# daovietanh190499/3D_Reconstruction

Measured on AMD Instinct MI355X. Metric: image-pairs matched/sec, higher is better.
Workload: dtype f32 descriptors: int8 MFMA certified filter + f64 re-score; 1 GPU; C3/C4 all-pairs BF-L2 + ratio 0.75: 257 imgs x 4096 kpts x 256-d, exact f32-input semantics (oracle.match.bf_match_exact, bit for bit); pairs=32896, api=dist.match_all_pairs_sharded(exact=True), match_mode=exact-float, parallelism=pairs/1

## Files before the change

### 3d_reconstruction_amd/csrc/match.hip

```cpp
#include "common.h"
#include <climits>
#include <cstdlib>

namespace sfmhip {

typedef int i32x4 __attribute__((ext_vector_type(4)));
typedef int i32x16 __attribute__((ext_vector_type(16)));

constexpr int kJB = 128;

template <int D>
__device__ __forceinline__ int swz_off(int r, int c) {
    constexpr int CPR = D / 16;
    constexpr int RPB = 256 / D;
    return r * D + ((c ^ ((r / RPB) % CPR)) << 4);
}

__device__ __forceinline__ int max3i(int a, int b, int c) {
    int r;
    asm("v_max3_i32 %0, %1, %2, %3" : "=v"(r) : "v"(a), "v"(b), "v"(c));
    return r;
}
__device__ __forceinline__ int med3i(int a, int b, int c) {
    int r;
    asm("v_med3_i32 %0, %1, %2, %3" : "=v"(r) : "v"(a), "v"(b), "v"(c));
    return r;
}

__global__ void quantize_kernel(const float* __restrict__ in, int64_t total, int d, int m_pad,
                                const int32_t* __restrict__ nk, int mode, int8_t* __restrict__ out) {
    const int64_t n4 = total >> 2;
    for (int64_t q = (int64_t)blockIdx.x * blockDim.x + threadIdx.x; q < n4;
         q += (int64_t)gridDim.x * blockDim.x) {
        const int64_t e = q << 2;
        const int64_t row = e / d;
        const int img = (int)(row / m_pad);
        const int r = (int)(row % m_pad);
        const float4 x = *reinterpret_cast<const float4*>(in + e);
        char4 o = make_char4(0, 0, 0, 0);
        if (r < nk[img]) {
            float v[4] = {x.x, x.y, x.z, x.w};
            int qv[4];
#pragma unroll
            for (int t = 0; t < 4; ++t) {
                if (mode == 0) {
                    float rr = fminf(fmaxf(__builtin_rintf(v[t]), 0.f), 255.f);
                    qv[t] = (int)rr - 128;
                } else {
                    float rr = __builtin_rintf(127.f * v[t]);
                    rr = fminf(fmaxf(rr, -127.f), 127.f);
                    qv[t] = (int)rr;
                }
            }
            o = make_char4((signed char)qv[0], (signed char)qv[1], (signed char)qv[2], (signed char)qv[3]);
        }
        *reinterpret_cast<char4*>(out + e) = o;
    }
}

__global__ void prepare_kernel(const int8_t* __restrict__ desc, int n_rows, int m_pad, int d,
                               const int32_t* __restrict__ nk, int32_t* __restrict__ norms,
                               int32_t* __restrict__ keys) {
    const int row = blockIdx.x * blockDim.x + threadIdx.x;
    if (row >= n_rows) return;
    const int img = row / m_pad, r = row % m_pad;
    const int8_t* p = desc + (size_t)row * d;
    int s = 0;
    for (int k = 0; k < d; k += 16) {
        const i32x4 v = *reinterpret_cast<const i32x4*>(p + k);
#pragma unroll
        for (int w = 0; w < 4; ++w) {
            const int x = v[w];
#pragma unroll
            for (int t = 0; t < 4; ++t) {
                const int q = (int)(signed char)((x >> (8 * t)) & 0xff);
                s += q * q;
            }
        }
    }
    norms[row] = s;
    const int low = 127 - (r & (kJB - 1));
    keys[row] = (r < nk[img]) ? (-s * 128 + low) : (INT_MIN + low);
}

__global__ void key_values_kernel(const int32_t* __restrict__ keys, int64_t n, int32_t* __restrict__ h,
                                  float* __restrict__ hf) {
    for (int64_t e = (int64_t)blockIdx.x * blockDim.x + threadIdx.x; e < n; e += (int64_t)gridDim.x * blockDim.x) {
        const int v = keys[e] >> 8;
        h[e] = v;
        if (hf) hf[e] = (float)v;
    }
}

__device__ __forceinline__ int fp6_grid_index(float y, int* g) {
    const float t = fminf(fabsf(y), 60.f);
    int n, m;
    if (t < 16.f) { m = (int)__builtin_rintf(t); n = m; }
    else if (t < 32.f) { const int r = (int)__builtin_rintf(0.5f * t); m = 2 * r; n = r + 8; }
    else { const int r = (int)__builtin_rintf(0.25f * t); m = 4 * r; n = r + 16; }
    const bool neg = y < 0.f && m > 0;
    *g = neg ? -m : m;
    return n | (neg ? 32 : 0);
}
__global__ void quantize_fp6_kernel(const float* __restrict__ in, int64_t n_chunks, int d, int m_pad,
                                    const int32_t* __restrict__ nk, int8_t* __restrict__ g,
                                    uint8_t* __restrict__ code) {
    for (int64_t c = (int64_t)blockIdx.x * blockDim.x + threadIdx.x; c < n_chunks;
         c += (int64_t)gridDim.x * blockDim.x) {
        const int64_t e0 = c * 32, row = e0 / d;
        const int img = (int)(row / m_pad), r = (int)(row % m_pad);
        const bool valid = r < nk[img];
        unsigned gw[8], cw[8];
#pragma unroll
        for (int w = 0; w < 8; ++w) gw[w] = cw[w] = 0u;
        if (valid) {
#pragma unroll
            for (int q = 0; q < 8; ++q) {
                const float4 x = *reinterpret_cast<const float4*>(in + e0 + 4 * q);
                const float v[4] = {x.x, x.y, x.z, x.w};
                unsigned pk = 0u;
#pragma unroll
                for (int t = 0; t < 4; ++t) {
                    int gv;
                    const int cd = fp6_grid_index(127.f * v[t], &gv);
                    gw[q] |= (unsigned)(gv & 0xff) << (8 * t);
                    pk |= (unsigned)cd << (6 * t);
                }
#pragma unroll
                for (int t = 0; t < 3; ++t) {
                    const int byte = 3 * q + t;
                    cw[byte >> 2] |= ((pk >> (8 * t)) & 0xffu) << (8 * (byte & 3));
                }
            }
        }
        uint4* go = reinterpret_cast<uint4*>(g + e0);
        uint4* co = reinterpret_cast<uint4*>(code + e0);
        go[0] = make_uint4(gw[0], gw[1], gw[2], gw[3]);
        go[1] = make_uint4(gw[4], gw[5], gw[6], gw[7]);
        co[0] = make_uint4(cw[0], cw[1], cw[2], cw[3]);
        co[1] = make_uint4(cw[4], cw[5], cw[6], cw[7]);
    }
}

template <int D, int WAVES>
struct Stager {
    static constexpr int CPR = D / 16;
    static constexpr int RPB = 256 / D;
    static constexpr int TILE = kJB * D;
    static constexpr int NI = TILE / 1024;
    static constexpr int PER_WAVE = NI / WAVES;
    static constexpr int LDT = TILE / 16 / (64 * WAVES);
    static_assert(NI % WAVES == 0 && LDT >= 1, "block / workgroup mismatch");

    __device__ static void dma(const int8_t* src, const int32_t* ksrc, int8_t* dst, int32_t* kdst, int wave,
                               int lane) {
#pragma unroll
        for (int u = 0; u < PER_WAVE; ++u) {
            const int ins = wave * PER_WAVE + u;
            const int rows_per_ins = 1024 / D;
            const int r0 = ins * rows_per_ins;
            const int r = r0 + lane / CPR;
            const int c = (lane % CPR) ^ ((r / RPB) % CPR);
            __builtin_amdgcn_global_load_lds(
                (__attribute__((address_space(1))) void*)(src + (size_t)r * D + c * 16),
                (__attribute__((address_space(3))) void*)(dst + r0 * D), 16, 0, 0);
        }
        if (wave == WAVES - 1) {
#pragma unroll
            for (int u = 0; u < 2; ++u)
                __builtin_amdgcn_global_load_lds(
                    (__attribute__((address_space(1))) void*)(ksrc + u * 64 + lane),
                    (__attribute__((address_space(3))) void*)(kdst + u * 64), 4, 0, 0);
        }
    }
};

template <int MF> struct Mfma;
template <> struct Mfma<32> {
    using acc_t = i32x16;
    static constexpr int NREG = 16, KB = 32;
    __device__ static acc_t run(i32x4 a, i32x4 b, acc_t c) {
        return __builtin_amdgcn_mfma_i32_32x32x32_i8(a, b, c, 0, 0, 0);
    }
    __device__ static int row(int q, int grp) { return (q & 3) + 8 * (q >> 2) + 4 * grp; }
};
template <> struct Mfma<16> {
    using acc_t = i32x4;
    static constexpr int NREG = 4, KB = 64;
    __device__ static acc_t run(i32x4 a, i32x4 b, acc_t c) {
        return __builtin_amdgcn_mfma_i32_16x16x64_i8(a, b, c, 0, 0, 0);
    }
    __device__ static int row(int q, int grp) { return 4 * grp + q; }
};

struct CertArgs {
    const double* erow;
    const double* eimg;
    double inv_s;
    int force;
};
constexpr int kUndecidedBase = -3;
constexpr int kValueOnlyTiles = 4;
__device__ __forceinline__ int sqrt8_ceil(int d2) {
    const long long t = 64LL * d2;
    int u = (int)ceil(sqrt((double)t));
    while (u > 0 && (long long)(u - 1) * (u - 1) >= t) --u;
    while ((long long)u * u < t) ++u;
    return u;
}
template <typename OutT>
__device__ __forceinline__ int undecided_mark(int d2) {
    if constexpr (sizeof(OutT) == 2) return kUndecidedBase - sqrt8_ceil(d2);
    else return kUndecidedBase - d2;
}
template <typename OutT>
__device__ __forceinline__ double mark_sqrt_d2(int mark) {
    if constexpr (sizeof(OutT) == 2) return (double)(kUndecidedBase - mark) * 0.125;
    else return sqrt((double)(kUndecidedBase - mark));
}

__device__ __forceinline__ int certify(int d1lo, int d1hi, int d2lo, int d2hi, double E, double inv_s, double rn2,
                                       double rd2) {
    const double up = 1.0 + 0x1p-50, dn = 1.0 - 0x1p-50;
    const double s1l = sqrt((double)d1lo) * inv_s, s1h = sqrt((double)d1hi) * inv_s;
    const double s2l = sqrt((double)d2lo) * inv_s, s2h = sqrt((double)d2hi) * inv_s;
    const double a1 = fmax(s1l * dn - E * up, 0.0), b1 = (s1h + E) * up;
    const double a2 = fmax(s2l * dn - E * up, 0.0), b2 = (s2h + E) * up;
    const double wl = 1.0 - 1e-12, wh = 1.0 + 1e-12;
    const double lo1 = a1 * a1 * wl, hi1 = b1 * b1 * wh, lo2 = a2 * a2 * wl, hi2 = b2 * b2 * wh;
    if (rd2 * lo1 >= rn2 * hi2) return 0;
    if (hi1 < lo2 && rd2 * hi1 < rn2 * lo2) return 1;
    return -1;
}

template <int D, int MF, int NS, int VG, typename OutT>
__device__ __forceinline__ void value_only_tail(const int (&w1)[NS], const int (&w2)[NS], const int (&wr)[NS],
                                                const int8_t* __restrict__ desc, const int8_t* __restrict__ bdesc,
                                                const int32_t* __restrict__ bkeys, const int32_t* __restrict__ norms,
                                                int a, int b, int m_pad, int na_rows, int ibase, int grp, int lr,
                                                int lane, long long rn2, long long rd2, OutT* __restrict__ out_m,
                                                const CertArgs& ca) {
    constexpr int NG = 64 / MF;
    int v1 = INT_MIN, v2 = INT_MIN, loc = 0;
#pragma unroll
    for (int s = 0; s < NS; ++s) {
        int a1 = w1[s], a2 = w2[s], al = wr[s] * NG + grp;
#pragma unroll
        for (int off = MF; off < 64; off <<= 1) {
            const int o1 = __shfl_xor(a1, off), o2 = __shfl_xor(a2, off), ol = __shfl_xor(al, off);
            const bool mine = a1 > o1 || (a1 == o1 && al < ol);
            a2 = max3i(min(a1, o1), a2, o2);
            al = mine ? al : ol;
            a1 = max(a1, o1);
        }
        if (s == grp) { v1 = a1; v2 = a2; loc = al; }
    }
    const int i = ibase + grp * MF + lr;
    int res = -1, na = 0, du1 = 0, hidx = -1;
    double E = 0.0;
    bool survivor = false;
    if (i < na_rows) {
        na = norms[(size_t)a * m_pad + i];
        du1 = na - 2 * v1;
        const int du2ub = na - 2 * v2;
        E = ca.erow[(size_t)a * m_pad + i] + ca.eimg[b];
        if (ca.force)
            res = undecided_mark<OutT>(min(du2ub, D * 255 * 255));
        else
            survivor = certify(max(du1 - 1, 0), du1, max(du1 - 1, 0), du2ub, E, ca.inv_s, (double)rn2,
                               (double)rd2) != 0;
    }
    constexpr int NC = 4 * VG;
    constexpr int LPC = (64 / NC) < (D / 16) ? (64 / NC) : (D / 16);
    constexpr int BPL = D / LPC;
    const int c = min(lane / LPC, NC - 1), part = lane % LPC;
    unsigned long long bal = __ballot(survivor);
    while (bal) {
        const int l = __builtin_ctzll(bal);
        bal &= bal - 1;
        const int ri = __shfl(i, l), rv = __shfl(v1, l), rl = __shfl(loc, l);
        const int j0 = (rl / NG) * VG * MF + 4 * (rl % NG);
        const int j = j0 + (c >> 2) * MF + (c & 3);
        const int8_t* pa = desc + ((size_t)a * m_pad + ri) * D + part * BPL;
        const int8_t* pb = bdesc + (size_t)j * D + part * BPL;
        int dot = 0;
#pragma unroll
        for (int w = 0; w < BPL / 16; ++w) {
            const i32x4 x = *reinterpret_cast<const i32x4*>(pa + 16 * w);
            const i32x4 y = *reinterpret_cast<const i32x4*>(pb + 16 * w);
#pragma unroll
            for (int e = 0; e < 4; ++e) dot = __builtin_amdgcn_sdot4(x[e], y[e], dot, false);
        }
#pragma unroll
        for (int off = 1; off < LPC; off <<= 1) dot += __shfl_xor(dot, off);
        const int u = dot + bkeys[j];
        const bool hit = lane < NC * LPC && part == 0 && u == rv;
        const unsigned long long hb = __ballot(hit);
        int x = u == rv ? INT_MIN : u;
#pragma unroll
        for (int off = LPC; off < 64; off <<= 1) x = max(x, __shfl_xor(x, off));
        if (lane == l) {
            const bool one = __popcll(hb) == 1;
            v2 = max(v2, one ? x : rv);
            if (one) {
                const int hc = __builtin_ctzll(hb) / LPC;
                hidx = j0 + (hc >> 2) * MF + (hc & 3);
            }
        }
    }
    if (survivor) {
        const int du2 = na - 2 * v2;
        const int v = certify(max(du1 - 1, 0), du1, max(du2 - 1, 0), du2, E, ca.inv_s, (double)rn2, (double)rd2);
        res = v == 0 ? -1 : (v > 0 && hidx >= 0) ? hidx : undecided_mark<OutT>(du2);
    }
    if (i < m_pad) out_m[i] = (OutT)res;
}

template <int D, int MF, int NS, int WAVES, bool CERT = false, typename OutT = int32_t, int VG = 0>
__global__ __launch_bounds__(64 * WAVES, 2) void match_kernel(
    const int8_t* __restrict__ desc, const int32_t* __restrict__ norms,
    const int32_t* __restrict__ keys, const int32_t* __restrict__ nk, int m_pad,
    const int32_t* __restrict__ pairs, int n_iblk, int nwg, long long rn2, long long rd2,
    OutT* __restrict__ m0, int32_t* __restrict__ dist1, int32_t* __restrict__ dist2, CertArgs ca) {
    using S = Stager<D, WAVES>;
    using M = Mfma<MF>;
    using acc_t = typename M::acc_t;
    constexpr int KK = D / M::KB;
    constexpr int CPK = M::KB / 16;
    constexpr int NG = 64 / MF;
    constexpr int TILE = S::TILE;
    constexpr int NT = 64 * WAVES;
    constexpr int IW = MF * NS;
    constexpr int IB = IW * WAVES;
    constexpr int JT = kJB / MF;
    static_assert(NS % NG == 0 || NG % NS == 0, "output lane mapping");
    constexpr bool VO = VG > 0;
    static_assert(!VO || (CERT && M::NREG == 4 && NS == NG && JT % VG == 0), "value-only form: 16x16 tiles, NS == NG");

    __shared__ __attribute__((aligned(16))) int8_t lds[2 * TILE + 2 * kJB * 4];

    const int wg = xcd_remap(blockIdx.x, nwg);
    const int pair = wg / n_iblk, ib = wg % n_iblk;
    const int a = pairs[2 * pair], b = pairs[2 * pair + 1];
    const int na_rows = nk[a], nb_rows = nk[b];
    const int tid = threadIdx.x, lane = tid & 63;
    const int wave = __builtin_amdgcn_readfirstlane(tid >> 6);
    const int grp = lane / MF, lr = lane % MF;
    const int ibase = ib * IB + wave * IW;
    OutT* out_m = m0 + (size_t)pair * m_pad;

    if (ib * IB >= na_rows || nb_rows < 2) {
        const int iend = min(ib * IB + IB, m_pad);
        for (int i = ib * IB + tid; i < iend; i += NT) {
            out_m[i] = -1;
            if (dist1) dist1[(size_t)pair * m_pad + i] = -1;
            if (dist2) dist2[(size_t)pair * m_pad + i] = -1;
        }
        return;
    }

    const int8_t* bdesc = desc + (size_t)b * m_pad * D;
    const int32_t* bkeys = keys + (size_t)b * m_pad;
    const int nblk = (nb_rows + kJB - 1) / kJB;
    int32_t* kbase = reinterpret_cast<int32_t*>(lds + 2 * TILE);

    S::dma(bdesc, bkeys, lds, kbase, wave, lane);

    i32x4 bq[NS][KK];
#pragma unroll
    for (int s = 0; s < NS; ++s) {
        const int i = min(ibase + s * MF + lr, m_pad - 1);
        const int8_t* rp = desc + ((size_t)a * m_pad + i) * D + grp * 16;
#pragma unroll
        for (int kk = 0; kk < KK; ++kk) bq[s][kk] = *reinterpret_cast<const i32x4*>(rp + kk * M::KB);
    }

    int g1k[NS], g1i[NS], g2k[NS], g1w[NS], g1b[NS];
#pragma unroll
    for (int s = 0; s < NS; ++s) { g1k[s] = INT_MIN; g1i[s] = 0; g1w[s] = 127; g1b[s] = 0; g2k[s] = INT_MIN; }
    int w1[NS], w2[NS], wr[NS];
#pragma unroll
    for (int s = 0; s < NS; ++s) { w1[s] = INT_MIN; w2[s] = INT_MIN; wr[s] = 0; }

    __syncthreads();

    for (int blk = 0; blk < nblk; ++blk) {
        const int cur = blk & 1;
        if (blk + 1 < nblk)
            S::dma(bdesc + (size_t)(blk + 1) * TILE, bkeys + (blk + 1) * kJB, lds + (cur ^ 1) * TILE,
                   kbase + (cur ^ 1) * kJB, wave, lane);
        const int8_t* tl = lds + cur * TILE;
        const int32_t* kl = kbase + cur * kJB;
        if constexpr (VO) {
            int rm[NS];
#pragma unroll
            for (int jt = 0; jt < JT; ++jt) {
                if (jt % VG == 0) {
#pragma unroll
                    for (int s = 0; s < NS; ++s) rm[s] = INT_MIN;
                }
                const i32x4 hv = *reinterpret_cast<const i32x4*>(kl + jt * MF + M::row(0, grp));
                acc_t acc[NS];
#pragma unroll
                for (int s = 0; s < NS; ++s) acc[s] = hv;
                const int r = jt * MF + lr;
#pragma unroll
                for (int kk = 0; kk < KK; ++kk) {
                    const i32x4 av = *reinterpret_cast<const i32x4*>(tl + swz_off<D>(r, kk * CPK + grp));
#pragma unroll
                    for (int s = 0; s < NS; ++s) acc[s] = M::run(av, bq[s][kk], acc[s]);
                }
#pragma unroll
                for (int s = 0; s < NS; ++s) {
                    rm[s] = max(max(rm[s], acc[s][0]), acc[s][1]);
                    rm[s] = max(max(rm[s], acc[s][2]), acc[s][3]);
                }
                if (jt % VG == VG - 1) {
                    const int rid = blk * (JT / VG) + jt / VG;
#pragma unroll
                    for (int s = 0; s < NS; ++s) {
                        wr[s] = rm[s] > w1[s] ? rid : wr[s];
                        w2[s] = med3i(w1[s], w2[s], rm[s]);
                        w1[s] = max(w1[s], rm[s]);
                    }
                }
            }
            __syncthreads();
            continue;
        }
        int t1[NS], t2[NS];
#pragma unroll
        for (int s = 0; s < NS; ++s) { t1[s] = INT_MIN; t2[s] = INT_MIN; }
#pragma unroll
        for (int jt = 0; jt < JT; ++jt) {
            acc_t acc[NS];
#pragma unroll
            for (int s = 0; s < NS; ++s) acc[s] = acc_t{0};
            const int r = jt * MF + lr;
#pragma unroll
            for (int kk = 0; kk < KK; ++kk) {
                const i32x4 av = *reinterpret_cast<const i32x4*>(tl + swz_off<D>(r, kk * CPK + grp));
#pragma unroll
                for (int s = 0; s < NS; ++s) acc[s] = M::run(av, bq[s][kk], acc[s]);
            }
#pragma unroll
            for (int g = 0; g < M::NREG / 4; ++g) {
                const i32x4 kv = *reinterpret_cast<const i32x4*>(kl + jt * MF + M::row(4 * g, grp));
#pragma unroll
                for (int e = 0; e < 4; e += 2) {
#pragma unroll
                    for (int s = 0; s < NS; ++s) {
                        const int ka = acc[s][4 * g + e] * 256 + kv[e];
                        const int kb = acc[s][4 * g + e + 1] * 256 + kv[e + 1];
                        const int m = med3i(t1[s], ka, kb);
                        t1[s] = max3i(t1[s], ka, kb);
                        t2[s] = max(t2[s], m);
                    }
                }
            }
        }
#pragma unroll
        for (int s = 0; s < NS; ++s) {
            if constexpr (D <= 128) {
                const int k1 = t1[s] >> 7, k2 = t2[s] >> 7;
                const bool up = k1 > g1k[s];
                g2k[s] = max3i(min(g1k[s], k1), g2k[s], k2);
                g1w[s] = up ? t1[s] : g1w[s];
                g1b[s] = up ? blk : g1b[s];
                g1k[s] = max(g1k[s], k1);
            } else {
                const int k1 = t1[s] >> 7, k2 = t2[s] >> 7, ix = blk * kJB + 127 - (t1[s] & 127);
                if (k1 > g1k[s]) { g2k[s] = max(g1k[s], k2); g1k[s] = k1; g1i[s] = ix; }
                else             { g2k[s] = max(g2k[s], k1); }
            }
        }
        __syncthreads();
    }

    if constexpr (VO) {
        value_only_tail<D, MF, NS, VG, OutT>(w1, w2, wr, desc, bdesc, bkeys, norms, a, b, m_pad, na_rows, ibase, grp, lr,
                                             lane, rn2, rd2, out_m, ca);
        return;
    }
    if constexpr (D <= 128) {
#pragma unroll
        for (int s = 0; s < NS; ++s) g1i[s] = g1b[s] * kJB + 127 - (g1w[s] & 127);
    }
#pragma unroll
    for (int s = 0; s < NS; ++s) {
#pragma unroll
        for (int off = MF; off < 64; off <<= 1) {
            const int ok = __shfl_xor(g1k[s], off), oi = __shfl_xor(g1i[s], off), o2 = __shfl_xor(g2k[s], off);
            const bool mine = (g1k[s] > ok) || (g1k[s] == ok && g1i[s] < oi);
            const int n2 = mine ? max(g2k[s], ok) : max(o2, g1k[s]);
            if (!mine) { g1k[s] = ok; g1i[s] = oi; }
            g2k[s] = n2;
        }
    }
#pragma unroll
    for (int s = 0; s < NS; ++s) {
        if (s % NG != grp % NS) continue;
        const int i = ibase + s * MF + lr;
        if (i >= m_pad) continue;
        int res = -1, d1 = -1, d2 = -1;
        if (i < na_rows) {
            const int na = norms[(size_t)a * m_pad + i];
            d1 = na - g1k[s];
            d2 = na - g2k[s];
            if (CERT) {
                const int v = ca.force ? -1
                                       : certify(d1, d1, d2, d2, ca.erow[(size_t)a * m_pad + i] + ca.eimg[b], ca.inv_s,
                                                 (double)rn2, (double)rd2);
                res = v > 0 ? g1i[s] : (v == 0 ? -1 : undecided_mark<OutT>(d2));
            } else if (rd2 * (long long)d1 < rn2 * (long long)d2) {
                res = g1i[s];
            }
        }
        out_m[i] = (OutT)res;
        if (dist1) dist1[(size_t)pair * m_pad + i] = d1;
        if (dist2) dist2[(size_t)pair * m_pad + i] = d2;
    }
}

typedef int i32x2 __attribute__((ext_vector_type(2)));
typedef int i32x8 __attribute__((ext_vector_type(8)));
typedef float f32x4 __attribute__((ext_vector_type(4)));

__global__ void pack_fp6_kernel(const uint8_t* __restrict__ code, int64_t n_chunks, int d,
                                uint8_t* __restrict__ dense) {
    const int spr = d / 32;
    for (int64_t c = (int64_t)blockIdx.x * blockDim.x + threadIdx.x; c < n_chunks;
         c += (int64_t)gridDim.x * blockDim.x) {
        const int64_t row = c / spr;
        const int s = (int)(c % spr);
        const uint4 lo = *reinterpret_cast<const uint4*>(code + c * 32);
        const uint2 hi = *reinterpret_cast<const uint2*>(code + c * 32 + 16);
        uint8_t* rp = dense + row * (3 * d / 4);
        *reinterpret_cast<uint4*>(rp + 16 * s) = lo;
        *reinterpret_cast<uint2*>(rp + d / 2 + 8 * s) = hi;
    }
}

template <int D, int WAVES>
struct DenseStager {
    static constexpr int ROW = 3 * D / 4, LB = D / 2, HB = D / 4;
    static constexpr int LO = kJB * LB, TILE = kJB * ROW;
    static constexpr int CPR = LB / 16, RPB = 256 / LB;
    static constexpr int UPR = HB / 16, RPH = 256 / HB;
    static constexpr int NLO = LO / 1024 / WAVES, NHI = (TILE - LO) / 1024 / WAVES;
    static_assert(NLO * WAVES * 1024 == LO && NHI * WAVES * 1024 == TILE - LO && NLO >= 1 && NHI >= 1,
                  "block / workgroup mismatch");
    static_assert(RPB * CPR == 16 && RPH * UPR == 16, "a 16-row tile covers every bank once");

    __device__ static int lo_sw(int r) { return ((((r & 15) + 4) >> 3) & 1) ^ ((r / RPB) % CPR); }
    __device__ static int hi_sw(int r) { return (r / RPH) % UPR; }
    __device__ static int lo_off(int r, int s) { return r * LB + ((s ^ lo_sw(r)) << 4); }
    __device__ static int hi_off(int r, int s) { return LO + r * HB + ((((s >> 1) ^ hi_sw(r)) << 4) | ((s & 1) << 3)); }

    __device__ static void dma(const uint8_t* src, const int32_t* ksrc, int8_t* dst, int32_t* kdst, int wave,
                               int lane) {
#pragma unroll
        for (int u = 0; u < NLO; ++u) {
            const int ins = wave * NLO + u;
            const int r = ins * (1024 / LB) + lane / CPR;
            const int c = (lane % CPR) ^ lo_sw(r);
            __builtin_amdgcn_global_load_lds(
                (__attribute__((address_space(1))) void*)(src + (size_t)r * ROW + c * 16),
                (__attribute__((address_space(3))) void*)(dst + ins * 1024), 16, 0, 0);
        }
#pragma unroll
        for (int u = 0; u < NHI; ++u) {
            const int ins = wave * NHI + u;
            const int r = ins * (1024 / HB) + lane / UPR;
            const int c = (lane % UPR) ^ hi_sw(r);
            __builtin_amdgcn_global_load_lds(
                (__attribute__((address_space(1))) void*)(src + (size_t)r * ROW + LB + c * 16),
                (__attribute__((address_space(3))) void*)(dst + LO + ins * 1024), 16, 0, 0);
        }
        if (wave == WAVES - 1) {
#pragma unroll
            for (int u = 0; u < 2; ++u)
                __builtin_amdgcn_global_load_lds(
                    (__attribute__((address_space(1))) void*)(ksrc + u * 64 + lane),
                    (__attribute__((address_space(3))) void*)(kdst + u * 64), 4, 0, 0);
        }
    }
};

__device__ __forceinline__ i32x2 lds_read_b64(const int8_t* p) {
    return *(const volatile __attribute__((address_space(3))) i32x2*)p;
}

struct Fp6Operand {
    i32x4 lo;
    i32x2 hi;
    __device__ i32x8 tuple() const { return i32x8{lo[0], lo[1], lo[2], lo[3], hi[0], hi[1], 0, 0}; }
};

constexpr int kFp6Tiles = 8;
constexpr int kFp6Waves = 4;

template <int D, typename OutT>
__global__ __launch_bounds__(64 * kFp6Waves, 2) void match_fp6_kernel(
    const uint8_t* __restrict__ dense, const int8_t* __restrict__ g, const int32_t* __restrict__ norms,
    const int32_t* __restrict__ h, const float* __restrict__ hf, const int32_t* __restrict__ nk, int m_pad,
    const int32_t* __restrict__ pairs, int n_iblk, int nwg, long long rn2, long long rd2,
    OutT* __restrict__ m0, CertArgs ca) {
    constexpr int MF = 16, NS = kFp6Tiles, WAVES = kFp6Waves, VG = kValueOnlyTiles;
    static_assert(D % 128 == 0, "one scaled MFMA takes 128 elements of k");
    static_assert(NS % 4 == 0, "value_only_tail takes four query tiles at a time");
    using S = DenseStager<D, WAVES>;
    constexpr int KK = D / 128;
    constexpr int TILE = S::TILE;
    constexpr int NT = 64 * WAVES;
    constexpr int IW = MF * NS, IB = IW * WAVES;
    constexpr int JT = kJB / MF;
    constexpr int kScale = (int)0x82828282;
    constexpr float kLow = -16777216.f;

    __shared__ __attribute__((aligned(16))) int8_t lds[2 * TILE + 2 * kJB * 4];

    const int wg = xcd_remap(blockIdx.x, nwg);
    const int pair = wg / n_iblk, ib = wg % n_iblk;
    const int a = pairs[2 * pair], b = pairs[2 * pair + 1];
    const int na_rows = nk[a], nb_rows = nk[b];
    const int tid = threadIdx.x, lane = tid & 63;
    const int wave = __builtin_amdgcn_readfirstlane(tid >> 6);
    const int grp = lane / MF, lr = lane % MF;
    const int ibase = ib * IB + wave * IW;
    OutT* out_m = m0 + (size_t)pair * m_pad;

    if (ib * IB >= na_rows || nb_rows < 2) {
        const int iend = min(ib * IB + IB, m_pad);
        for (int i = ib * IB + tid; i < iend; i += NT) out_m[i] = -1;
        return;
    }

    const uint8_t* bdense = dense + (size_t)b * m_pad * S::ROW;
    const int32_t* bhf = reinterpret_cast<const int32_t*>(hf) + (size_t)b * m_pad;
    const int nblk = (nb_rows + kJB - 1) / kJB;
    int32_t* kbase = reinterpret_cast<int32_t*>(lds + 2 * TILE);

    S::dma(bdense, bhf, lds, kbase, wave, lane);

    Fp6Operand bq[NS][KK];
#pragma unroll
    for (int s = 0; s < NS; ++s) {
        const int i = min(ibase + s * MF + lr, m_pad - 1);
        const uint8_t* rp = dense + ((size_t)a * m_pad + i) * S::ROW;
#pragma unroll
        for (int kk = 0; kk < KK; ++kk) {
            bq[s][kk].lo = *reinterpret_cast<const i32x4*>(rp + 16 * (kk * 4 + grp));
            bq[s][kk].hi = *reinterpret_cast<const i32x2*>(rp + S::LB + 8 * (kk * 4 + grp));
        }
    }
    int lo_b[KK], hi_b[KK];
#pragma unroll
    for (int kk = 0; kk < KK; ++kk) {
        lo_b[kk] = S::lo_off(lr, kk * 4 + grp);
        hi_b[kk] = S::hi_off(lr, kk * 4 + grp);
    }

    float w1[NS], w2[NS];
    int wr[NS];
#pragma unroll
    for (int s = 0; s < NS; ++s) { w1[s] = kLow; w2[s] = kLow; wr[s] = 0; }

    __syncthreads();

    for (int blk = 0; blk < nblk; ++blk) {
        const int cur = blk & 1;
        if (blk + 1 < nblk)
            S::dma(bdense + (size_t)(blk + 1) * TILE, bhf + (blk + 1) * kJB, lds + (cur ^ 1) * TILE,
                   kbase + (cur ^ 1) * kJB, wave, lane);
        const int8_t* tl = lds + cur * TILE;
        const float* kl = reinterpret_cast<const float*>(kbase + cur * kJB);
        float rm[NS];
#pragma unroll
        for (int jt = 0; jt < JT; ++jt) {
            if (jt % VG == 0) {
#pragma unroll
                for (int s = 0; s < NS; ++s) rm[s] = kLow;
            }
            const f32x4 hv = *reinterpret_cast<const f32x4*>(kl + jt * MF + 4 * grp);
            f32x4 acc[NS];
#pragma unroll
            for (int s = 0; s < NS; ++s) acc[s] = hv;
#pragma unroll
            for (int kk = 0; kk < KK; ++kk) {
                Fp6Operand av;
                av.lo = *reinterpret_cast<const i32x4*>(tl + lo_b[kk] + jt * MF * S::LB);
                av.hi = lds_read_b64(tl + hi_b[kk] + jt * MF * S::HB);
#pragma unroll
                for (int s = 0; s < NS; ++s)
                    acc[s] = __builtin_amdgcn_mfma_scale_f32_16x16x128_f8f6f4(av.tuple(), bq[s][kk].tuple(), acc[s], 2, 2,
                                                                              0, kScale, 0, kScale);
            }
#pragma unroll
            for (int s = 0; s < NS; ++s) {
                rm[s] = __builtin_fmaxf(__builtin_fmaxf(rm[s], acc[s][0]), acc[s][1]);
                rm[s] = __builtin_fmaxf(__builtin_fmaxf(rm[s], acc[s][2]), acc[s][3]);
            }
            if (jt % VG == VG - 1) {
                const int rid = blk * (JT / VG) + jt / VG;
#pragma unroll
                for (int s = 0; s < NS; ++s) {
                    const bool up = rm[s] > w1[s];
                    wr[s] = up ? rid : wr[s];
                    w2[s] = __builtin_amdgcn_fmed3f(w1[s], w2[s], rm[s]);
                    w1[s] = up ? rm[s] : w1[s];
                }
            }
        }
        __syncthreads();
    }

#pragma unroll
    for (int q = 0; q < NS / 4; ++q) {
        int v1[4], v2[4], vr[4];
#pragma unroll
        for (int s = 0; s < 4; ++s) { v1[s] = (int)w1[4 * q + s]; v2[s] = (int)w2[4 * q + s]; vr[s] = wr[4 * q + s]; }
        value_only_tail<D, MF, 4, VG, OutT>(v1, v2, vr, g, g + (size_t)b * m_pad * D, h + (size_t)b * m_pad, norms, a, b,
                                            m_pad, na_rows, ibase + q * 4 * MF, grp, lr, lane, rn2, rd2, out_m, ca);
    }
}

__global__ void mutual_kernel(int32_t* __restrict__ m0, int32_t* __restrict__ m1, int P, int m_pad) {
    const int64_t total = (int64_t)P * m_pad;
    for (int64_t e = (int64_t)blockIdx.x * blockDim.x + threadIdx.x; e < total;
         e += (int64_t)gridDim.x * blockDim.x) {
        const int64_t base = (e / m_pad) * m_pad;
        const int i = (int)(e - base);
        const int j0 = m0[e];
        const int j1 = m1[e];
        const bool keep0 = j0 >= 0 && m1[base + j0] == i;
        const bool keep1 = j1 >= 0 && m0[base + j1] == i;
        if (j0 >= 0 && !keep0) m0[e] = -1;
        if (j1 >= 0 && !keep1) m1[e] = -1;
    }
}

constexpr int kVqObsPerBlock = 16;
constexpr int kVqCodesPerChunk = 32;

__global__ __launch_bounds__(256) void vq_kernel(const double* __restrict__ obs, int64_t n_obs,
                                                 const double* __restrict__ code, int n_codes, int d,
                                                 int32_t* __restrict__ codes, double* __restrict__ dist) {
    extern __shared__ double smem[];
    double* sobs = smem;
    double* scode = smem + kVqObsPerBlock * d;
    const int ld = d + 1;
    const int64_t o0 = (int64_t)blockIdx.x * kVqObsPerBlock;
    for (int t = threadIdx.x; t < kVqObsPerBlock * d; t += blockDim.x) {
        const int64_t o = o0 + t / d;
        sobs[t] = (o < n_obs) ? obs[o * d + (t % d)] : 0.0;
    }
    const int lo = threadIdx.x >> 4, l16 = threadIdx.x & 15;
    const double* x = sobs + lo * d;
    double best = __builtin_inf();
    int bidx = INT_MAX;
    for (int c0 = 0; c0 < n_codes; c0 += kVqCodesPerChunk) {
        const int nc = min(kVqCodesPerChunk, n_codes - c0);
        __syncthreads();
        for (int t = threadIdx.x; t < nc * d; t += blockDim.x) {
            const int r = t / d;
            scode[r * ld + (t - r * d)] = code[(size_t)(c0 + r) * d + (t - r * d)];
        }
        __syncthreads();
        double acc[2] = {0.0, 0.0};
        for (int k = 0; k < d; ++k) {
            const double xv = x[k];
#pragma unroll
            for (int j = 0; j < 2; ++j) {
                const int r = l16 + 16 * j;
                const double df = xv - scode[r * ld + k];
                acc[j] = __builtin_fma(df, df, acc[j]);
            }
        }
#pragma unroll
        for (int j = 0; j < 2; ++j) {
            const int r = l16 + 16 * j;
            if (r < nc && acc[j] < best) { best = acc[j]; bidx = c0 + r; }
        }
    }
#pragma unroll
    for (int off = 8; off >= 1; off >>= 1) {
        const double ob = __shfl_xor(best, off, 16);
        const int oi = __shfl_xor(bidx, off, 16);
        if (ob < best || (ob == best && oi < bidx)) { best = ob; bidx = oi; }
    }
    const int64_t o = o0 + lo;
    if (l16 == 0 && o < n_obs) {
        codes[o] = bidx;
        dist[o] = sqrt(best);
    }
}

typedef double v4d __attribute__((ext_vector_type(4)));
constexpr int kVqmWaves = 8;
constexpr int kVqmObsPerWave = 32;
constexpr int kVqmTile = kVqmWaves * kVqmObsPerWave;

template <int DP, bool FULL>
__global__ __launch_bounds__(kVqmWaves * 64) void vq_mfma_kernel(
    const double* __restrict__ obs, int64_t n_obs, const double* __restrict__ code, int n_codes, int d,
    int codes_per_pass, int32_t* __restrict__ codes, double* __restrict__ dist) {
    constexpr int LD = DP + 4;
    constexpr int KS = DP / 4;
    extern __shared__ double smem[];
    double* sc = smem;
    double* sn = smem + (size_t)codes_per_pass * LD;
    const int lane = threadIdx.x & 63, wave = threadIdx.x >> 6;
    const int r16 = lane & 15, kq = lane >> 4;
    const int64_t n_tiles = (n_obs + kVqmTile - 1) / kVqmTile;
    for (int c0 = 0; c0 < n_codes; c0 += codes_per_pass) {
        const int nc = min(codes_per_pass, n_codes - c0);
        const int ncb = (nc + 15) >> 4;
        const bool first = c0 == 0, last = c0 + codes_per_pass >= n_codes;
        __syncthreads();
        for (int t = threadIdx.x; t < ncb * 16 * DP; t += blockDim.x) {
            const int r = t / DP, k = t - r * DP;
            sc[r * LD + k] = (r < nc && (FULL || k < d)) ? code[(size_t)(c0 + r) * d + k] : 0.0;
        }
        __syncthreads();
        for (int r = threadIdx.x; r < ncb * 16; r += blockDim.x) {
            double s = 0.0;
            for (int k = 0; k < DP; ++k) s = __builtin_fma(sc[r * LD + k], sc[r * LD + k], s);
            sn[r] = r < nc ? s : __builtin_inf();
        }
        __syncthreads();
        for (int64_t t = blockIdx.x; t < n_tiles; t += gridDim.x) {
            const int64_t ob = t * kVqmTile + wave * kVqmObsPerWave;
            double a[2][KS];
#pragma unroll
            for (int h = 0; h < 2; ++h) {
                const int64_t o = ob + 16 * h + r16;
                const double* xp = obs + o * d;
#pragma unroll
                for (int s = 0; s < KS; ++s) {
                    const int k = 4 * s + kq;
                    a[h][s] = (o < n_obs && (FULL || k < d)) ? __builtin_nontemporal_load(xp + k) : 0.0;
                }
            }
            double best[2][4];
            int bj[2][4];
#pragma unroll
            for (int h = 0; h < 2; ++h)
#pragma unroll
                for (int g = 0; g < 4; ++g) { best[h][g] = __builtin_inf(); bj[h][g] = INT_MAX; }
            auto epilogue = [&](const v4d& acc0, const v4d& acc1, int j) {
                const double cn = sn[j];
#pragma unroll
                for (int g = 0; g < 4; ++g) {
                    const double d0 = cn - 2.0 * acc0[g];
                    const double d1 = cn - 2.0 * acc1[g];
                    if (d0 < best[0][g]) { best[0][g] = d0; bj[0][g] = c0 + j; }
                    if (d1 < best[1][g]) { best[1][g] = d1; bj[1][g] = c0 + j; }
                }
            };
            for (int cb = 0; cb < ncb; ++cb) {
                const int j = cb * 16 + r16;
                const double* bp = sc + j * LD + kq;
                v4d acc0 = {0.0, 0.0, 0.0, 0.0}, acc1 = {0.0, 0.0, 0.0, 0.0};
#pragma unroll
                for (int s = 0; s < KS; ++s) {
                    const double b = bp[4 * s];
                    acc0 = __builtin_amdgcn_mfma_f64_16x16x4f64(a[0][s], b, acc0, 0, 0, 0);
                    acc1 = __builtin_amdgcn_mfma_f64_16x16x4f64(a[1][s], b, acc1, 0, 0, 0);
                }
                epilogue(acc0, acc1, j);
            }
#pragma unroll
            for (int h = 0; h < 2; ++h) {
                int win = 0;
#pragma unroll
                for (int g = 0; g < 4; ++g) {
                    double bv = best[h][g];
                    int bi = bj[h][g];
#pragma unroll
                    for (int off = 8; off >= 1; off >>= 1) {
                        const double ov = __shfl_xor(bv, off, 16);
                        const int oi = __shfl_xor(bi, off, 16);
                        if (ov < bv || (ov == bv && oi < bi)) { bv = ov; bi = oi; }
                    }
                    const int64_t o = ob + 16 * h + kq + 4 * g;
                    if (!first && o < n_obs) {
                        const double prev = dist[o];
                        if (!(bv < prev)) { bv = prev; bi = codes[o]; }
                    }
                    if (!last && r16 == 0 && o < n_obs) {
                        codes[o] = bi;
                        dist[o] = bv;
                    }
                    const int w = __shfl(bi, (r16 & 3) * 16);
                    if ((r16 >> 2) == g) win = w;
                }
                if (last) {
                    const int64_t o = ob + 16 * h + r16;
                    const double* cp = code + (size_t)win * d;
                    double part = 0.0;
#pragma unroll
                    for (int s = 0; s < KS; ++s) {
                        const int k = 4 * s + kq;
                        const double df = a[h][s] - ((o < n_obs && (FULL || k < d)) ? cp[k] : 0.0);
                        part = __builtin_fma(df, df, part);
                    }
                    part += __shfl_xor(part, 16);
                    part += __shfl_xor(part, 32);
                    if (kq == 0 && o < n_obs) {
                        codes[o] = win;
                        dist[o] = sqrt(part);
                    }
                }
            }
        }
    }
}


typedef float f32x4 __attribute__((ext_vector_type(4)));
__device__ __forceinline__ double vq_eps_abs(int DP, double xn, double cmax) {
    return 0x1p-126 * (2.0 * sqrt((double)DP) * (cmax + xn) + 2.0 * DP + 4.0) * 1.01;
}
typedef double f64x2 __attribute__((ext_vector_type(2)));
typedef _Float16 f16x8 __attribute__((ext_vector_type(8)));
constexpr int kVqhWaves = 8;
__device__ __forceinline__ double vq_eps16(int DP, double xn, double cmax) {
    const double u = 0x1p-24;
    return 1.01 * (2.0 * xn * cmax * (0x1.8p-21 + 2.02 * DP * u + 4.0 * u) + 4.0 * u * cmax * cmax +
                   0x1p-24 * sqrt((double)DP) * (xn + cmax) + 2.0 * DP * 0x1p-48) +
           vq_eps_abs(DP, xn, cmax);
}
__device__ __forceinline__ int vqh_k(int j, int e, int q) { return 16 * (j & 7) + 4 * q + 2 * (j >> 3) + e; }
__device__ __forceinline__ double vqh_xor8(double v) {
    const int lo = __builtin_amdgcn_mov_dpp((int)__double2loint(v), 0x128, 0xF, 0xF, false);
    const int hi = __builtin_amdgcn_mov_dpp((int)__double2hiint(v), 0x128, 0xF, 0xF, false);
    return __hiloint2double(hi, lo);
}
template <int PROBE>
__global__ __launch_bounds__(kVqhWaves * 64) void vq_f16s_kernel(const double* __restrict__ obs, int64_t n_obs,
                                                                  const double* __restrict__ code, int n_codes,
                                                                  int32_t* __restrict__ codes,
                                                                  double* __restrict__ dist,
                                                                  unsigned* __restrict__ amb,
                                                                  unsigned* __restrict__ namb) {
    constexpr int DP = 128, KB = 4, KS = 32;
    extern __shared__ f32x4 smh[];
    const int ncb = (n_codes + 15) >> 4;
    const int ncp = (ncb + 1) & ~1;
    f16x8* sc = reinterpret_cast<f16x8*>(smh);
    float* sn = reinterpret_cast<float*>(smh + ncp * KB * 2 * 64);
    __shared__ unsigned s_cmax, s_big;
    const int lane = threadIdx.x & 63, wave = __builtin_amdgcn_readfirstlane(threadIdx.x >> 6);
    const int r16 = lane & 15, kq = lane >> 4;
    const bool b3 = (lane >> 3) & 1;
    if (threadIdx.x == 0) { s_cmax = 0u; s_big = 0u; }
    __syncthreads();
    for (int t = threadIdx.x; t < ncp * KB * 64; t += blockDim.x) {
        const int ln = t & 63, kb = (t >> 6) % KB, cb = t / (KB * 64);
        const int j = cb * 16 + (ln & 15);
        f16x8 hi, lo;
        bool big = false;
#pragma unroll
        for (int e = 0; e < 8; ++e) {
            const double v = j < n_codes ? code[(size_t)j * DP + vqh_k(4 * kb + (e >> 1), e & 1, ln >> 4)] : 0.0;
            big |= !(fabs(v) < 32768.0);
            const _Float16 h = (_Float16)(float)v;
            hi[e] = h;
            lo[e] = (_Float16)(float)(v - (double)h);
        }
        if (big) s_big = 1u;
        sc[((cb * KB + kb) * 2 + 0) * 64 + ln] = hi;
        sc[((cb * KB + kb) * 2 + 1) * 64 + ln] = lo;
    }
    for (int r = threadIdx.x; r < ncp * 16; r += blockDim.x) {
        double q = 0.0;
        if (r < n_codes)
            for (int k = 0; k < DP; ++k) q = __builtin_fma(code[(size_t)r * DP + k], code[(size_t)r * DP + k], q);
        sn[r] = r < n_codes ? (float)q : __builtin_inff();
        if (r < n_codes) atomicMax(&s_cmax, __float_as_uint((float)sqrt(q) * 1.001f));
    }
    __syncthreads();
    const double cmax = (double)__uint_as_float(s_cmax);
    const bool book_big = s_big != 0u;
    const int64_t n_units = (n_obs + 15) >> 4;
    const int64_t ustep = (int64_t)gridDim.x * kVqhWaves;
    f64x2 nx[KS / 2];
    auto fetch = [&](int64_t un) {
#pragma unroll
        for (int j = 0; j < KS / 2; ++j) {
            const f64x2* xp = reinterpret_cast<const f64x2*>(
                                  obs + min(un * 16 + (lane & 7) + 8 * (j >> 3), n_obs - 1) * DP) +
                              8 * (j & 7) + 2 * kq + b3;
            nx[j] = PROBE == 1 ? f64x2{(double)(lane + un) * 0x1p-10, (double)j * 0x1p-10}
                               : __builtin_nontemporal_load(xp);
        }
    };
    fetch(min((int64_t)blockIdx.x * kVqhWaves + wave, n_units - 1));
    for (int64_t un = (int64_t)blockIdx.x * kVqhWaves + wave; un < n_units; un += ustep) {
        const int64_t o = un * 16 + r16;
        double x[KS];
#pragma unroll
        for (int m = 0; m < 8; ++m) {
            const f64x2 a0 = nx[m], a1 = nx[8 + m];
            const double s0 = vqh_xor8(b3 ? a0.x : a1.x), s1 = vqh_xor8(b3 ? a0.y : a1.y);
            x[2 * m] = b3 ? s0 : a0.x;
            x[2 * m + 1] = b3 ? s1 : a0.y;
            x[16 + 2 * m] = b3 ? a1.x : s0;
            x[16 + 2 * m + 1] = b3 ? a1.y : s1;
        }
        fetch(min(un + ustep, n_units - 1));
        double xn = 0.0;
        bool big = book_big;
#pragma unroll
        for (int s = 0; s < KS; ++s) {
            xn = __builtin_fma(x[s], x[s], xn);
            big |= !(fabs(x[s]) < 32768.0);
        }
// ... 994 lines not shown
```

Baseline: 610,200 pairs/s.

## Software-pipeline FP6 MFMA loop with interleaved max reduction and merge steps

Restructures the fp6 matching inner loop into a hand-scheduled software pipeline. The next LDS operand and bias are prefetched during the current MFMAs, and each tile's max-reduction is split into two halves that are slotted between later MFMAs. The running top-2 merge is split into four single steps, with a compile-time schedule spreading them through the gaps of the following range. Per-lane DMA offsets are also precomputed once and source pointers advanced incrementally, removing address arithmetic from each block. The aim is to hide VALU and LDS latency behind MFMA issue, at the cost of extra live registers, scheduling barriers that restrict the compiler, and fragile schedule bookkeeping.

Measured after the change: 632,100 pairs/s (median of 6 runs). +3.6%, better.

```diff
diff --git a/3d_reconstruction_amd/csrc/fp6_sched.h b/3d_reconstruction_amd/csrc/fp6_sched.h
--- /dev/null
+++ b/3d_reconstruction_amd/csrc/fp6_sched.h
@@ -0,0 +1,51 @@
+#pragma once
+
+namespace sfmhip {
+
+template <int KK, int NS>
+struct Fp6Sched {
+    static constexpr int MPT = KK * NS;
+    static constexpr int F = (KK - 1) * NS + 5;
+    static constexpr int kBudget = KK == 1 ? 3 : 2;
+    static_assert(F + 1 < MPT, "a spilled maximum reads its chain before the next tile rewrites it");
+    static constexpr int chain(int g, int which) { return (g - F - which + MPT) % MPT; }
+    static constexpr bool back(int g, int which) { return g - F - which < 0; }
+    static constexpr int load(int g) { return (chain(g, 0) < NS) + (chain(g, 1) < NS); }
+    static constexpr int before(int g, int which) {
+        const int f = F + which, wrap = f + NS - MPT;
+        return (g < wrap ? g : wrap) + (g > f ? g - f : 0);
+    }
+    static constexpr int merge(int h, int j) {
+        const int g = h % MPT;
+        const int k = (h / MPT) * (kBudget * MPT - 2 * NS) + kBudget * g - before(g, 0) - before(g, 1);
+        return (j < kBudget - load(g) && k + j < 4 * NS) ? k + j : -1;
+    }
+    static constexpr int merge_chain(int k) { return 2 * (k / 8) + ((0xCA >> (k % 8)) & 1); }
+    static constexpr int merge_step(int k) { return (0x3232'1100 >> (4 * (k % 8))) & 15; }
+    static constexpr int kOwedFirst = MPT - F, kOwedSecond = MPT - F - 1;
+    static constexpr bool merge_ready() {
+        for (int c = 0; c < NS; ++c) {
+            int h = 0;
+            while (true) {
+                bool found = false;
+                for (int j = 0; j < kBudget; ++j) found |= merge(h, j) == 8 * (c / 2) + c % 2;
+                if (found) break;
+                ++h;
+            }
+            if (h < F + 1 + c - MPT) return false;
+        }
+        return true;
+    }
+};
+
+__device__ __forceinline__ void fp6_merge_step(int step, float m, int rid, bool& up, float& w1, float& w2, int& wr) {
+    const float a = w1, b = w2;
+    const int r = wr;
+    const bool u = up;
+    if (step == 0) up = m > a;
+    else if (step == 1) w2 = __builtin_amdgcn_fmed3f(a, b, m);
+    else if (step == 2) wr = u ? rid : r;
+    else w1 = u ? m : a;
+}
+
+}
diff --git a/3d_reconstruction_amd/csrc/match.hip b/3d_reconstruction_amd/csrc/match.hip
--- a/3d_reconstruction_amd/csrc/match.hip
+++ b/3d_reconstruction_amd/csrc/match.hip
@@ -1,4 +1,5 @@
 #include "common.h"
+#include "fp6_sched.h"
 #include <climits>
 #include <cstdlib>
 
@@ -557,31 +558,48 @@
     __device__ static int lo_off(int r, int s) { return r * LB + ((s ^ lo_sw(r)) << 4); }
     __device__ static int hi_off(int r, int s) { return LO + r * HB + ((((s >> 1) ^ hi_sw(r)) << 4) | ((s & 1) << 3)); }
 
+    struct Lanes {
+        unsigned lo[NLO], hi[NHI], key;
+    };
+    __device__ static Lanes lanes(int wave, int lane) {
+        Lanes l;
+#pragma unroll
+        for (int u = 0; u < NLO; ++u) {
+            const int r = (wave * NLO + u) * (1024 / LB) + lane / CPR;
+            l.lo[u] = (unsigned)(r * ROW + (((lane % CPR) ^ lo_sw(r)) << 4));
+        }
+#pragma unroll
+        for (int u = 0; u < NHI; ++u) {
+            const int r = (wave * NHI + u) * (1024 / HB) + lane / UPR;
+            l.hi[u] = (unsigned)(r * ROW + LB + (((lane % UPR) ^ hi_sw(r)) << 4));
+        }
+        l.key = (unsigned)(lane * 4);
+        return l;
+    }
+
     __device__ static void dma(const uint8_t* src, const int32_t* ksrc, int8_t* dst, int32_t* kdst, int wave,
-                               int lane) {
+                               const Lanes& l) {
 #pragma unroll
         for (int u = 0; u < NLO; ++u) {
-            const int ins = wave * NLO + u;
-            const int r = ins * (1024 / LB) + lane / CPR;
-            const int c = (lane % CPR) ^ lo_sw(r);
+            unsigned o = l.lo[u];
+            asm volatile("" : "+v"(o));
+            __builtin_amdgcn_global_load_lds((__attribute__((address_space(1))) void*)(src + o),
+                                             (__attribute__((address_space(3))) void*)(dst + (wave * NLO + u) * 1024),
+                                             16, 0, 0);
+        }
+#pragma unroll
+        for (int u = 0; u < NHI; ++u) {
+            unsigned o = l.hi[u];
+            asm volatile("" : "+v"(o));
             __builtin_amdgcn_global_load_lds(
-                (__attribute__((address_space(1))) void*)(src + (size_t)r * ROW + c * 16),
-                (__attribute__((address_space(3))) void*)(dst + ins * 1024), 16, 0, 0);
-        }
-#pragma unroll
-        for (int u = 0; u < NHI; ++u) {
-            const int ins = wave * NHI + u;
-            const int r = ins * (1024 / HB) + lane / UPR;
-            const int c = (lane % UPR) ^ hi_sw(r);
-            __builtin_amdgcn_global_load_lds(
-                (__attribute__((address_space(1))) void*)(src + (size_t)r * ROW + LB + c * 16),
-                (__attribute__((address_space(3))) void*)(dst + LO + ins * 1024), 16, 0, 0);
+                (__attribute__((address_space(1))) void*)(src + o),
+                (__attribute__((address_space(3))) void*)(dst + LO + (wave * NHI + u) * 1024), 16, 0, 0);
         }
         if (wave == WAVES - 1) {
 #pragma unroll
             for (int u = 0; u < 2; ++u)
                 __builtin_amdgcn_global_load_lds(
-                    (__attribute__((address_space(1))) void*)(ksrc + u * 64 + lane),
+                    (__attribute__((address_space(1))) void*)(reinterpret_cast<const uint8_t*>(ksrc + u * 64) + l.key),
                     (__attribute__((address_space(3))) void*)(kdst + u * 64), 4, 0, 0);
         }
     }
@@ -611,6 +629,10 @@
     static_assert(NS % 4 == 0, "value_only_tail takes four query tiles at a time");
     using S = DenseStager<D, WAVES>;
     constexpr int KK = D / 128;
+    using SC = Fp6Sched<KK, NS>;
+    static_assert(kJB / MF == 2 * VG, "two ranges per block: the range maxima alternate between two sets");
+    static_assert(SC::merge(VG * SC::MPT, 0) == -1, "a range's gaps hold the previous range's merge");
+    static_assert(SC::merge_ready(), "a chain's merge starts behind its last maximum");
     constexpr int TILE = S::TILE;
     constexpr int NT = 64 * WAVES;
     constexpr int IW = MF * NS, IB = IW * WAVES;
@@ -641,7 +663,8 @@
     const int nblk = (nb_rows + kJB - 1) / kJB;
     int32_t* kbase = reinterpret_cast<int32_t*>(lds + 2 * TILE);
 
-    S::dma(bdense, bhf, lds, kbase, wave, lane);
+    const typename S::Lanes dl = S::lanes(wave, lane);
+    S::dma(bdense, bhf, lds, kbase, wave, dl);
 
     Fp6Operand bq[NS][KK];
 #pragma unroll
@@ -663,57 +686,96 @@
 
     float w1[NS], w2[NS];
     int wr[NS];
-#pragma unroll
-    for (int s = 0; s < NS; ++s) { w1[s] = kLow; w2[s] = kLow; wr[s] = 0; }
+    f32x4 acc[NS];
+    float half[NS], rm[2][NS];
+    bool up[NS];
+    int rid_owed = 0;
+#pragma unroll
+    for (int s = 0; s < NS; ++s) {
+        w1[s] = kLow; w2[s] = kLow; wr[s] = 0;
+        acc[s] = f32x4{kLow, kLow, kLow, kLow};
+        half[s] = rm[0][s] = rm[1][s] = kLow;
+        up[s] = false;
+    }
+    auto merge_step = [&](int c, int step, float m, int rid) {
+        fp6_merge_step(step, m, rid, up[c], w1[c], w2[c], wr[c]);
+    };
 
     __syncthreads();
 
+    const uint8_t* bsrc = bdense;
+    const int32_t* ksrc = bhf;
     for (int blk = 0; blk < nblk; ++blk) {
         const int cur = blk & 1;
+        bsrc += TILE;
+        ksrc += kJB;
         if (blk + 1 < nblk)
-            S::dma(bdense + (size_t)(blk + 1) * TILE, bhf + (blk + 1) * kJB, lds + (cur ^ 1) * TILE,
-                   kbase + (cur ^ 1) * kJB, wave, lane);
+            S::dma(bsrc, ksrc, lds + (cur ^ 1) * TILE, kbase + (cur ^ 1) * kJB, wave, dl);
         const int8_t* tl = lds + cur * TILE;
         const float* kl = reinterpret_cast<const float*>(kbase + cur * kJB);
-        float rm[NS];
+        Fp6Operand av;
+        av.lo = *reinterpret_cast<const i32x4*>(tl + lo_b[0]);
+        av.hi = lds_read_b64(tl + hi_b[0]);
+        f32x4 hv = *reinterpret_cast<const f32x4*>(kl + 4 * grp);
 #pragma unroll
         for (int jt = 0; jt < JT; ++jt) {
-            if (jt % VG == 0) {
-#pragma unroll
-                for (int s = 0; s < NS; ++s) rm[s] = kLow;
-            }
-            const f32x4 hv = *reinterpret_cast<const f32x4*>(kl + jt * MF + 4 * grp);
-            f32x4 acc[NS];
-#pragma unroll
-            for (int s = 0; s < NS; ++s) acc[s] = hv;
+            const int R = jt / VG, tt = jt % VG;
+            f32x4 hv_n = hv;
 #pragma unroll
             for (int kk = 0; kk < KK; ++kk) {
-                Fp6Operand av;
-                av.lo = *reinterpret_cast<const i32x4*>(tl + lo_b[kk] + jt * MF * S::LB);
-                av.hi = lds_read_b64(tl + hi_b[kk] + jt * MF * S::HB);
-#pragma unroll
-                for (int s = 0; s < NS; ++s)
-                    acc[s] = __builtin_amdgcn_mfma_scale_f32_16x16x128_f8f6f4(av.tuple(), bq[s][kk].tuple(), acc[s], 2, 2,
-                                                                              0, kScale, 0, kScale);
-            }
-#pragma unroll
-            for (int s = 0; s < NS; ++s) {
-                rm[s] = __builtin_fmaxf(__builtin_fmaxf(rm[s], acc[s][0]), acc[s][1]);
-                rm[s] = __builtin_fmaxf(__builtin_fmaxf(rm[s], acc[s][2]), acc[s][3]);
-            }
-            if (jt % VG == VG - 1) {
-                const int rid = blk * (JT / VG) + jt / VG;
+                Fp6Operand av_n = av;
+                __builtin_amdgcn_sched_barrier(0);
 #pragma unroll
                 for (int s = 0; s < NS; ++s) {
-                    const bool up = rm[s] > w1[s];
-                    wr[s] = up ? rid : wr[s];
-                    w2[s] = __builtin_amdgcn_fmed3f(w1[s], w2[s], rm[s]);
-                    w1[s] = up ? rm[s] : w1[s];
+                    acc[s] = __builtin_amdgcn_mfma_scale_f32_16x16x128_f8f6f4(av.tuple(), bq[s][kk].tuple(),
+                                                                              kk == 0 ? hv : acc[s], 2, 2, 0, kScale, 0,
+                                                                              kScale);
+                    __builtin_amdgcn_sched_barrier(0);
+                    if (s == 0) {
+                        if (kk + 1 < KK) {
+                            av_n.lo = *reinterpret_cast<const i32x4*>(tl + lo_b[kk + 1] + jt * MF * S::LB);
+                            av_n.hi = lds_read_b64(tl + hi_b[kk + 1] + jt * MF * S::HB);
+                        } else if (jt + 1 < JT) {
+                            av_n.lo = *reinterpret_cast<const i32x4*>(tl + lo_b[0] + (jt + 1) * MF * S::LB);
+                            av_n.hi = lds_read_b64(tl + hi_b[0] + (jt + 1) * MF * S::HB);
+                            hv_n = *reinterpret_cast<const f32x4*>(kl + (jt + 1) * MF + 4 * grp);
+                        }
+                        __builtin_amdgcn_sched_barrier(0);
+                    }
+                    const int gp = kk * NS + s;
+                    if (const int c = SC::chain(gp, 0); c < NS) {
+                        const int of = tt - SC::back(gp, 0);
+                        const float from = of < 0 ? rm[R ^ 1][c] : of == 0 ? kLow : rm[R][c];
+                        half[c] = __builtin_fmaxf(__builtin_fmaxf(from, acc[c][0]), acc[c][1]);
+                    }
+                    if (const int c = SC::chain(gp, 1); c < NS)
+                        rm[tt == 0 && SC::back(gp, 1) ? R ^ 1 : R][c] =
+                            __builtin_fmaxf(__builtin_fmaxf(half[c], acc[c][2]), acc[c][3]);
+#pragma unroll
+                    for (int j = 0; j < SC::kBudget; ++j)
+                        if (const int k = SC::merge(tt * SC::MPT + gp, j); k >= 0) {
+                            __builtin_amdgcn_sched_barrier(0);
+                            merge_step(SC::merge_chain(k), SC::merge_step(k), rm[R ^ 1][SC::merge_chain(k)], rid_owed);
+                        }
+                    __builtin_amdgcn_sched_barrier(0);
                 }
-            }
+                av = av_n;
+            }
+            hv = hv_n;
+            if (tt == VG - 1) rid_owed = blk * (JT / VG) + R;
         }
         __syncthreads();
     }
+#pragma unroll
+    for (int s = SC::kOwedFirst; s < NS; ++s)
+        half[s] = __builtin_fmaxf(__builtin_fmaxf(rm[1][s], acc[s][0]), acc[s][1]);
+#pragma unroll
+    for (int s = SC::kOwedSecond; s < NS; ++s)
+        rm[1][s] = __builtin_fmaxf(__builtin_fmaxf(half[s], acc[s][2]), acc[s][3]);
+#pragma unroll
+    for (int s = 0; s < NS; ++s)
+#pragma unroll
+        for (int step = 0; step < 4; ++step) merge_step(s, step, rm[1][s], rid_owed);
 
 #pragma unroll
     for (int q = 0; q < NS / 4; ++q) {
```
